# colmap/privacy_preserving_sfm

Hardware: AMD Instinct MI355X
Metric: BA iterations/sec + RANSAC hypotheses/sec, 500 cams / 200k line obs (higher is better)
Workload: dtype f64; 1 GPU; configs[2]: 500 cams / 200k line obs full BA (K1+K2+K3, MFMA Schur solve) on 1xMI355X; cams=500, points=25000, obs=200000, camera_model=SIMPLE_RADIAL, reduced_system=3000, successful_steps=2561, lm_chunk=10, submodels=1, exchange=none (independent sub-models), linear_solver=cholesky (one launch: chain workgroup + task list), cholesky_fallbacks=0

## Files before the change

### privacy_preserving_sfm_amd/csrc/chol_plan.hpp

```cpp
#pragma once
#include <algorithm>
#include <cmath>
#include <cstdint>
#include <cstdio>
#include <cstring>
#include <initializer_list>
#include <utility>
#include <vector>

#include "switches.hpp"

#ifdef __HIPCC__
#define PP_PLAN_HD __host__ __device__ __forceinline__
#else
#define PP_PLAN_HD inline
#endif

namespace ppsfm {

constexpr int kMaxChains = 16;
struct ChainRanges { int32_t n; int32_t begin[kMaxChains]; int32_t end[kMaxChains]; int32_t post[kMaxChains]; };
inline ChainRanges OneChain(int T) { ChainRanges cr; std::memset(&cr, 0, sizeof(cr)); cr.n = 1; cr.end[0] = T; return cr; }

PP_PLAN_HD void TriIndex(int t, int* row, int* col) {
  int r = (int)((sqrt(8.0 * t + 1.0) - 1.0) * 0.5);
  while ((r + 1) * (r + 2) / 2 <= t) ++r;
  while (r * (r + 1) / 2 > t) --r;
  *row = r; *col = t - r * (r + 1) / 2;
}

constexpr int BacksubNumPairs(int T) { return T >= 7 ? (T - 3) / 2 : 0; }

constexpr int kMaxSteps = 128;
constexpr int kMaxSuper = kMaxSteps / 2 + 1;
constexpr int kScratchCounters = 2048;
enum { cSol0 = 8, cVer0 = cSol0 + kMaxChains * kMaxSteps, cSub0 = cVer0 + kMaxSuper * kMaxSuper, cScratch0 = cSub0 + kMaxSuper * kMaxSuper,
       kNumCounters = cScratch0 + kScratchCounters };
static_assert(kNumCounters * sizeof(int32_t) <= 8192 * sizeof(double), "counters exceed their part of the workspace (CholeskyWorkspaceDoubles)");
enum { kTaskPrepX = 1, kTaskPrepD = 2, kTaskSolve = 3, kTaskUpdate = 4, kTaskPairPrep = 5, kTaskMerge = 6 };
struct ChainTask { int32_t type, k, a, b, w0, w1, w2, flags, cidx, sidx, zsel, mask, slot[4]; };
constexpr int TaskSuperColumn(int32_t b) { return b & 255; }
constexpr int TaskPart(int32_t b) { return (b >> 8) & 15; }
constexpr int TaskParts(int32_t b) { return (b >> 12) & 15; }
constexpr int TaskTarget(int32_t b) { return b >> 16; }
constexpr bool TaskFirstOfChain(int32_t flags) { return (flags & 1) != 0; }
constexpr int TaskChain(int32_t flags) { return (flags >> 4) & 15; }
constexpr int32_t PackUpdate(int J, int part, int parts, int target) { return J | (part << 8) | (parts << 12) | (target << 16); }
constexpr int32_t PackFlags(bool first, int chain) { return (first ? 1 : 0) | (chain << 4); }
constexpr int kPartsTwoPanels = 8;
constexpr double kUpdateSlope = 0.3;
inline int WholeFrom(int T) { return T >= 56 ? 2 : 3; }

constexpr bool StepOwnsTile(int k, int r, int c) { return (r == k + 1 && c == k + 1) || (r == k + 2 && (c == k + 1 || c == k + 2)); }

inline int CloseTileMap(int T, uint8_t* nz) {
  for (int i = 0; i < T; ++i) nz[(size_t)i * T + i] = 1;
  std::vector<int> rows;
  for (int k = 0; k < T; ++k) {
    rows.clear();
    for (int i = k + 1; i < T; ++i) if (nz[(size_t)i * T + k]) rows.push_back(i);
    for (size_t a = 0; a < rows.size(); ++a)
      for (size_t b = 0; b <= a; ++b) nz[(size_t)rows[a] * T + rows[b]] = 1;
  }
  int count = 0;
  for (int i = 0; i < T; ++i) for (int j = 0; j <= i; ++j) count += nz[(size_t)i * T + j] ? 1 : 0;
  return count;
}

struct SparseColumnLists { std::vector<int32_t> lists; int base_rows = 0, base_sups = 0; };
inline SparseColumnLists BuildSparseColumnLists(int T, const uint8_t* nz) {
  auto has = [&](int i, int j) { return i < T && j < T && nz[(size_t)i * T + j] != 0; };
  std::vector<int32_t> rows, sups, row_off(T + 1, 0), sup_off(T + 1, 0);
  for (int k = 0; k + 1 < T; ++k) {
    row_off[k] = (int32_t)rows.size(); sup_off[k] = (int32_t)sups.size();
    for (int i = k + 3; i < T; ++i) if (has(i, k)) rows.push_back(i);
    if (k >= 1) {
      const int kp = k - 1, k1 = kp + 2, nb = T - k1, ns = (nb + 1) / 2, nsup = ns * (ns + 1) / 2 - 1;
      for (int u = 0; u < nsup; ++u) {
        int I, J;
        TriIndex(u + 1, &I, &J);
        bool any = false;
        for (int q = 0; q < 4; ++q) {
          const int bi = k1 + 2 * I + (q >> 1), bj = k1 + 2 * J + (q & 1);
          any = any || (bi < T && bj < T && bi >= bj && has(bi, kp) && has(bj, kp));
// ... 46 lines not shown
  }
  if (nz) {
    p.map.assign(nz, nz + (size_t)T * T);
    for (int c = 0; c < p.cr.n; ++c)
      for (int k = p.cr.begin[c]; k < p.cr.end[c]; ++k)
        for (int i = k; i < p.cr.end[c] && i <= k + 2; ++i) p.map[(size_t)i * T + k] = 1;
    (void)CloseTileMap(T, p.map.data());
  }
  p.time.assign(T, 0);
  for (int k = 0; k < T; ++k) {
    int t = 0;
    const int ck = p.chain_of[k];
    for (int j = 0; j < k; ++j) {
      if (!nz) { t = std::max(t, p.time[j] + 1); continue; }
      if (p.chain_of[j] == ck) { if (p.map[(size_t)k * T + j]) t = std::max(t, p.time[j] + 1); continue; }
      for (int r = k; r <= k + 2 && r < p.cr.end[ck]; ++r) if (p.map[(size_t)r * T + j]) t = std::max(t, p.time[p.cr.end[p.chain_of[j]] - 1] + 2);
    }
    p.time[k] = t;
  }
  std::vector<int> order(T);
  for (int k = 0; k < T; ++k) order[k] = k;
  std::stable_sort(order.begin(), order.end(), [&](int a, int b) { return p.time[a] < p.time[b]; });
  p.rho1.assign(T, 0);
  for (int r = 0; r < T; ++r) p.rho1[order[r]] = r + 1;
  for (int c = 0; c < p.cr.n; ++c) p.cr.post[c] = p.cr.end[c] < T ? p.rho1[p.cr.end[c] - 2] : 0;
  return p;
}

struct TaskListInfo { bool fits = true; int scratch_tiles = 0; };
class TaskListBuilder {
 public:
  TaskListBuilder(int T, const ChainPlan& plan, const PlanSwitches& ps)
      : T(T), plan(plan), nz(plan.Map()), nch(plan.cr.n), whole_from(ps.whole_from ? *ps.whole_from : WholeFrom(T)), two_panels(!nz && ps.two_panels),
        slope(ps.slope ? *ps.slope : kUpdateSlope), time(plan.time), rho1(plan.rho1), own(kMaxSuper * kMaxSuper), scratch(nch),
        solpost((size_t)nch * (T + 4), 0), rowkey((size_t)nch * (T + 4), kNone), tilekey((size_t)(T + 4) * (T + 4), kNone), stepkey(T + 4, kNone) {
    for (int I = 0; I < kMaxSuper; ++I) for (int J = 0; J < kMaxSuper; ++J) { own[I * kMaxSuper + J].cidx = cVer0 + I * kMaxSuper + J; own[I * kMaxSuper + J].sidx = cSub0 + I * kMaxSuper + J; }
  }

  std::vector<ChainTask> Build(TaskListInfo* info) {
    struct Event { int t, kind, k; };
    std::vector<Event> events;
    for (int k = 0; k + 1 < T; ++k) events.push_back({time[k], 0, k});
    for (int c = 0; c + 1 < nch; ++c) events.push_back({time[plan.cr.end[c] - 1] + 1, 1, plan.cr.end[c]});
    std::stable_sort(events.begin(), events.end(), [](const Event& a, const Event& b) { return a.t != b.t ? a.t < b.t : (a.kind != b.kind ? a.kind < b.kind : a.k < b.k); });
    for (const Event& ev : events) {
      if (ev.kind == 1) { ListUpdates(ev.k, ev.t, true); ListMerges(plan.chain_of[ev.k - 1], ev.t); continue; }
      ListChainStep(ev.k);
      if (ev.k != plan.cr.begin[plan.chain_of[ev.k]]) ListUpdates(ev.k, time[ev.k], false);
    }
    if (!nz)
      for (int gp = 0; gp < BacksubNumPairs(T); ++gp)
        for (int part = 0; part < (gp + 1 < BacksubNumPairs(T) ? 3 : 1); ++part) items.push_back({2 * gp + 2.2, {kTaskPairPrep, 2 * gp + 2, gp, part, 0, 0, 0, 0, 0, 0, -1, 0, {0, 0, 0, 0}}});
    std::stable_sort(items.begin(), items.end(), [](const Item& a, const Item& b) { return a.key < b.key; });
    std::vector<ChainTask> list(items.size());
    for (size_t i = 0; i < items.size(); ++i) list[i] = items[i].t;
    if (info) { info->fits = ok; info->scratch_tiles = slots_used; }
    return list;
  }

 private:
  static constexpr double kNone = -1e30;
  struct Item { double key; ChainTask t; };
  struct Seq { int cidx = 0, sidx = 0, listed = 0, post = 0, touched = 0; double key = -1e30; int slot[4] = {-1, -1, -1, -1}; };

  const int T;
  const ChainPlan& plan;
  const uint8_t* const nz;
  const int nch, whole_from;
  const bool two_panels;
  const double slope;
  const std::vector<int>& time;
  const std::vector<int>& rho1;
  std::vector<Seq> own;
  std::vector<std::vector<std::pair<int, Seq>>> scratch;
  int scratch_used = 0, slots_used = 0;
  bool ok = true;
  std::vector<int> solpost;
  std::vector<double> rowkey;
  std::vector<double> tilekey;
  std::vector<double> stepkey;
  std::vector<Item> items;

  bool Has(int i, int j) const { return i < T && j < T && (!nz || nz[(size_t)i * T + j] != 0); }
  double& TileKey(int r, int c) { return tilekey[(size_t)r * (T + 4) + c]; }
  int& SolPost(int c, int row) { return solpost[(size_t)c * (T + 4) + row]; }
  double& RowKey(int c, int row) { return rowkey[(size_t)c * (T + 4) + row]; }
  int VerPost(int I, int J) const { return own[I * kMaxSuper + J].post; }
  double VerKey(int I, int J) const { return own[I * kMaxSuper + J].key; }
  static double Raised(double desired, std::initializer_list<double> deps) { double k = desired; for (double d : deps) k = std::max(k, d); return k; }
  int Owner(int J) const { return plan.chain_of[std::min(2 * J, T - 1)]; }
  Seq& SeqOf(int c, int I, int J) {
    if (c == Owner(J)) return own[I * kMaxSuper + J];
    for (auto& e : scratch[c]) if (e.first == I * kMaxSuper + J) return e.second;
    Seq q;
    if (scratch_used + 2 > kScratchCounters) ok = false; else { q.cidx = cScratch0 + scratch_used; q.sidx = cScratch0 + scratch_used + 1; scratch_used += 2; }
    scratch[c].push_back({I * kMaxSuper + J, q});
    return scratch[c].back().second;
  }
  double OperandKey(double dep, int k, int I, int J, int col, bool if_nz) {
    for (int row : {2 * I, 2 * I + 1, 2 * J, 2 * J + 1})
      if (row < T && row >= k + 1 && (!if_nz || Has(row, col))) dep = std::max(dep, TileKey(row, col));
    return dep;
// ... 21 lines not shown
      SolPost(c, k + 1) = rho1[k];
    }
    for (int i = k + 3; i < T; ++i)
      if (Has(i, k)) {
        const double key = Raised(tk - 0.3, {VerKey(i >> 1, k >> 1), RowKey(c, i), step_prev});
        items.push_back({key, {kTaskSolve, k, i, 0, VerPost(i >> 1, k >> 1), rho1[k], SolPost(c, i), fl, 0, 0, -1, 0, {0, 0, 0, 0}}});
        SolPost(c, i) = rho1[k]; TileKey(i, k) = key; RowKey(c, i) = key;
      }
  }

  int CoupledTiles(int k, int I, int J) const {
    int tiles = 0;
    for (int q = 0; q < 4; ++q) {
      const int bi = 2 * I + (q >> 1), bj = 2 * J + (q & 1);
      if (bi < T && bj < T && bi >= bj && bj >= k + 1 && !StepOwnsTile(k, bi, bj) && Has(bi, k - 1) && Has(bj, k - 1)) tiles |= 1 << q;
    }
    return tiles;
  }

  void ListUpdates(int k, int ts, bool pseudo) {
    const int pc = plan.chain_of[k - 1], fl = PackFlags(false, pc);
    for (int J = (k + 1) / 2; 2 * J < T; ++J)
      for (int I = J; 2 * I < T; ++I) {
        const int tiles = CoupledTiles(k, I, J);
        if (!tiles) continue;
        Seq& sq = SeqOf(pc, I, J);
        const bool into_scratch = pc != Owner(J);
        const int zsel = into_scratch ? pc : -1;
        double dep = OperandKey(sq.key, k, I, J, k - 1, true);
        const int tJ = std::min(time[2 * J], 2 * J + 1 < T ? time[2 * J + 1] : time[2 * J]);
        const int Jt = std::max(tJ / 2, (ts + 1) / 2);
        const bool front = !pseudo && I == (k + 3) / 2 && (J == I - 1 || J == I);
        const bool far = Jt - (ts + 1) / 2 >= whole_from;
        const bool far_next = two_panels && k + 2 < T && J - (k + 2) / 2 >= whole_from;
        if (far && (k & 1) == 0 && two_panels) continue;
        if (far && far_next && (k & 1) == 1) {
          sq.listed += 1;
          dep = OperandKey(dep, k, I, J, k, false);
          const double key = Raised((k + 1) + slope * (J - 0.5 * (k + 2)), {dep});
          items.push_back({key, {kTaskUpdate, k, I, PackUpdate(J, 0, kPartsTwoPanels, sq.listed), sq.post, k + 1, k, 0, sq.cidx, sq.sidx, -1, 0, {0, 0, 0, 0}}});
          sq.post = k + 1; sq.key = key;
          continue;
        }
        const int parts = front ? 4 : (far ? 1 : 2);
        sq.listed += parts;
        const double dist = std::max(0.5 * tJ - 0.5 * (ts + 1), -0.5);
        const double key = Raised(front ? ts - 0.2 : ts + slope * dist, {dep});
        const int post = std::max(rho1[k - 1], sq.post + 1);
        const int fresh = into_scratch ? (tiles & ~sq.touched) : 0;
        if (into_scratch) for (int q = 0; q < 4; ++q) if (((fresh >> q) & 1) && sq.slot[q] < 0) sq.slot[q] = slots_used++;
        for (int q = 0; q < parts; ++q)
          items.push_back({key, {kTaskUpdate, k, I, PackUpdate(J, q, parts, sq.listed), sq.post, post, rho1[k - 1], fl, sq.cidx, sq.sidx, zsel, fresh,
                                 {sq.slot[0], sq.slot[1], sq.slot[2], sq.slot[3]}}});
        sq.post = post; sq.key = key; sq.touched |= tiles;
      }
  }

  void ListMerges(int c, int ts) {
    for (auto& e : scratch[c]) {
      const int I = e.first / kMaxSuper, J = e.first % kMaxSuper;
      Seq& z = e.second;
      Seq& o = own[e.first];
      const double key = Raised(ts + 0.05, {z.key, o.key});
      const int post = o.post + 1;
      items.push_back({key, {kTaskMerge, plan.cr.end[c], I, PackUpdate(J, 0, 0, 0), o.post, post, z.post, 0, o.cidx, z.cidx, c, z.touched, {z.slot[0], z.slot[1], z.slot[2], z.slot[3]}}});
      o.post = post; o.key = key;
    }
  }
};
inline std::vector<ChainTask> BuildTaskList(int T, const ChainPlan& plan, const PlanSwitches& ps, TaskListInfo* info = nullptr) {
  return TaskListBuilder(T, plan, ps).Build(info);
}

class TaskListReplay {
// ... 90 lines not shown
    const int I = t.a, J = TaskSuperColumn(t.b), c = t.zsel;
    if (c < 0 || c >= nch || t.cidx != cVer0 + I * kMaxSuper + J) return false;
    if (ctr[t.cidx] < t.w0 || ctr[t.sidx] < t.w2) return false;
    for (int q = 0; q < 4; ++q) {
      const int r = 2 * I + (q >> 1), cc = 2 * J + (q & 1);
      if (r >= T || cc >= T) { if ((t.mask >> q) & 1) return false; continue; }
      Bits& z = zapplied[c][(size_t)r * T + cc];
      if (((t.mask >> q) & 1) != (z.none() ? 0 : 1)) return false;
      if (!z.none() && t.slot[q] != zslot[c][(size_t)r * T + cc]) return false;
      Bits& a = Applied(r, cc);
      if ((a.w[0] & z.w[0]) || (a.w[1] & z.w[1])) return false;
      a.w[0] |= z.w[0]; a.w[1] |= z.w[1];
      z = Bits();
    }
    if (ctr[t.cidx] >= t.w1) return false;
    ctr[t.cidx] = t.w1;
    return true;
  }

  bool ScratchSlotIsOwn(const ChainTask& t, int q, int r, int c) {
    int& zs = zslot[t.zsel][(size_t)r * T + c];
    if (t.slot[q] < 0) return false;
    if (zs < 0) {
      if ((int)slot_taken.size() <= t.slot[q]) slot_taken.resize(t.slot[q] + 1, 0);
      if (slot_taken[t.slot[q]]) return false;
      slot_taken[t.slot[q]] = 1; zs = t.slot[q];
    } else if (zs != t.slot[q]) return false;
    return true;
  }

  bool Update(const ChainTask& t) {
    const int k = t.k, fc = TaskChain(t.flags);
    const int I = t.a, J = TaskSuperColumn(t.b), part = TaskPart(t.b), parts = TaskParts(t.b), target = TaskTarget(t.b);
    const bool two = parts == kPartsTwoPanels;
    if (fc != plan.chain_of[k - 1] || t.zsel >= nch || (t.zsel >= 0 && t.zsel != fc)) return false;
    if (t.zsel < 0 && (t.cidx != cVer0 + I * kMaxSuper + J || t.sidx != cSub0 + I * kMaxSuper + J)) return false;
    if (ctr[t.cidx] < t.w0) return false;
    auto row_ok = [&](int row, bool distinct) {
      if (!(distinct && row < T && row >= k + 1 && Has(row, k - 1))) return true;
      int have = Sol(fc, row);
      if (ChainStores(row, k - 1)) have = std::max(have, plan.cr.post[fc]);
      return have >= (two ? t.w2 + 1 : t.w2);
    };
    const int bi = 2 * I + (parts == 2 ? part : part >> 1), bj0 = 2 * J + (parts == 2 ? 0 : part & 1), nb = parts == 2 ? 2 : 1;
    bool rows_ok;
    if (parts == 1 || two) rows_ok = row_ok(2 * I, true) && row_ok(2 * I + 1, true) && row_ok(2 * J, J != I) && row_ok(2 * J + 1, J != I);
    else rows_ok = row_ok(bi, true) && row_ok(bj0, bj0 != bi) && row_ok(bj0 + 1, nb == 2 && bj0 + 1 != bi);
    if (!rows_ok) return false;
    for (int q = 0; q < 4; ++q) {
      const int r = 2 * I + (q >> 1), c = 2 * J + (q & 1);
      const bool mine = (parts == 1 || two) || (parts == 2 ? (q >> 1) == part : q == part);
      for (int kk = k; kk <= (two ? k + 1 : k); ++kk) {
        const bool valid = r < T && c < T && r >= c && c >= kk + 1 && !StepOwnsTile(kk, r, c) && Has(r, kk - 1) && Has(c, kk - 1);
        if (!mine || !valid) continue;
        for (int row : {r, c}) if (!Solved(row, kk - 1) && !ChainStores(row, kk - 1) && !(two && kk == k + 1)) return false;
        if ((t.zsel < 0) != (plan.chain_of[kk - 1] == plan.chain_of[c])) return false;
        Bits& a = t.zsel < 0 ? Applied(r, c) : zapplied[t.zsel][(size_t)r * T + c];
        if (t.zsel >= 0 && (((t.mask >> q) & 1) != (a.none() ? 1 : 0))) return false;
        if (t.zsel >= 0 && !ScratchSlotIsOwn(t, q, r, c)) return false;
        if (a.w[(kk - 1) >> 6] >> ((kk - 1) & 63) & 1) return false;
        SetBit(&a, kk - 1);
      }
    }
    if (++ctr[t.sidx] == target) {
      if (ctr[t.cidx] >= t.w1) return false;
      ctr[t.cidx] = t.w1;
    }
    return true;
  }

  bool Complete() {
    for (int c = 0; c + 1 < T; ++c)
      for (int r = c + 1; r < T; ++r) {
        if (!Has(r, c)) continue;
        const int e = plan.cr.end[plan.chain_of[c]];
        if (r == c + 1 && r < e) { if (!Solved(r, c) && !(c + 2 >= e && CanRun(c))) return false; }
        else if (!Solved(r, c)) return false;
      }
    for (int c = 1; c < T; ++c)
      for (int r = c; r < T; ++r) {
        for (int ch = 0; ch < nch; ++ch) if (!zapplied[ch][(size_t)r * T + c].none()) return false;
        if (!Has(r, c)) continue;
        Bits want = Coupling(r, c, c);
        auto clear = [&](int p) { if (p >= 0) want.w[p >> 6] &= ~(1ull << (p & 63)); };
        clear(c - 1); if (r <= c + 1) clear(c - 2); if (r == c) clear(c - 3);
        if (!(Applied(r, c) == want)) return false;
      }
    return true;
// ... 31 lines not shown
```

### privacy_preserving_sfm_amd/csrc/cholesky.hip

```cpp
#include <algorithm>
#include <chrono>
#include <cmath>
#include <cstdio>
#include <cstdlib>
#include <cstring>
#include <mutex>
#include <string>
#include <type_traits>
#include <utility>
#include <vector>

#include "ba_impl.hpp"
#include "chol_block.hpp"
#include "chol_plan.hpp"
#include "resource_pool.hpp"

namespace ppsfm {

__global__ __launch_bounds__(kPanelThreads) void k_potrf64(double* __restrict__ S, int ld, double* __restrict__ Minv, double* __restrict__ xs, int32_t* __restrict__ flag,
                                                           double* __restrict__ x_out, double* Lout, int32_t* __restrict__ ctr, int nctr, double* mail,
                                                           long long mail_doubles, ChainRanges cr) {
  __shared__ __attribute__((aligned(16))) double smem[2 * kNB * kLS];
  __shared__ double inv_diag[kNB];
  double* A = smem;
// ... 695 lines not shown
  TileStoreD(PP_TILE(Bc, s, ct), x, lr, g);
  if (kIsX) {
#pragma unroll
    for (int r = 0; r < 4; ++r) StoreThrough(L + row_k2 + col_k + (size_t)(16 * s + g + 4 * r) * ld + 16 * ct + lr, x[r]);
    if (!FetchMailTile<true>(Ba, mb.xsol + (size_t)k * kNB * kNB, tid, flag, s_failed)) return;
    TaskStoresDone();
    if (tid == 0) __hip_atomic_store(ctr + solbase + (k + 2), done_k, __ATOMIC_RELAXED, __HIP_MEMORY_SCOPE_AGENT);
    out = UpdateTileRegs(out, Bc, Ba, ti, tj, lr, g);
    double* mail = mb.xs + (size_t)(k + 1) * kNB * kNB;
#pragma unroll
    for (int i = 0; i < 4; ++i) StoreMail(mail + (16 * ti + g + 4 * i) * kNB + 16 * tj + lr, out[i]);
    PP_TASK_MAX(5, k);
    StoreTile(L + row_k1 + col_k, Ba, ld, tid);
    TaskStoresDone();
    if (tid == 0) __hip_atomic_store(ctr + solbase + (k + 1), done_k, __ATOMIC_RELAXED, __HIP_MEMORY_SCOPE_AGENT);
  } else {
    __syncthreads();
    double* mail = mb.ds + (size_t)(k + 1) * kNB * kNB;
    if (has_out) {
      out = UpdateTileRegs(out, Bc, Bc, di, dj, lr, g);
#pragma unroll
      for (int i = 0; i < 4; ++i) StoreMail(mail + (16 * di + g + 4 * i) * kNB + 16 * dj + lr, out[i]);
    } else {
      int ui = 0, uj = 1, rem = w - 10;
      while (rem >= 3 - ui) { rem -= 3 - ui; ++ui; }
      uj = ui + 1 + rem;
#pragma unroll
      for (int i = 0; i < 4; ++i) StoreThrough(mail + (16 * ui + g + 4 * i) * kNB + 16 * uj + lr, 0.0);
    }
    PP_TASK_MAX(6, k);
  }
}

template <bool kTwo>
__device__ __forceinline__ void UpdateSuperTile(double* S, const double* L, int ld, int kp, int T, int I, int J, double* As, double* Bs, const uint8_t* __restrict__ nz, int fresh_mask = 0, double* zpool = nullptr, const int32_t* slot = nullptr) {
  const int tid = threadIdx.x, lane = tid & 63, w = tid >> 6;
  const int lr = lane & 15, lk = lane >> 4;
  const int wi = w >> 2, wj = w & 3;
  const int k = kp + 1, bi0 = 2 * I, bj0 = 2 * J;
  const int bi = bi0 + (wi >> 1), bj = bj0 + (wj >> 1);
  const bool front = (bi == k + 1 && bj == k + 1) || (bi == k + 2 && (bj == k + 1 || bj == k + 2));
  bool valid = bi < T && bj < T && bi >= bj && bj >= k + 1 && !front;
  if (valid && nz) valid = nz[(size_t)bi * T + kp] && nz[(size_t)bj * T + kp];
  const size_t cbase = (size_t)bi * kNB * ld + (size_t)bj * kNB + (size_t)(32 * (wi & 1) + lk) * ld + 32 * (wj & 1) + lr;
  const v4f64 z = (v4f64){0.0, 0.0, 0.0, 0.0};
  v4f64 c[2][2], p[2][2] = {{z, z}, {z, z}};
  const size_t col = (size_t)kp * kNB;
  const int ra1 = bi0 + 1 < T ? bi0 + 1 : bi0, rb1 = bj0 + 1 < T ? bj0 + 1 : bj0;
  const double* s0 = L + (size_t)bi0 * kNB * ld + col; const double* s1 = L + (size_t)ra1 * kNB * ld + col;
  const double* s2 = L + (size_t)bj0 * kNB * ld + col; const double* s3 = L + (size_t)rb1 * kNB * ld + col;
  LoadTiles4(As, s0, As + kNB * kLS, s1, Bs, s2, Bs + kNB * kLS, s3, ld, tid);
  const int tq = 2 * (wi >> 1) + (wj >> 1);
  const bool fresh = (fresh_mask >> tq) & 1;
  double* Cw = S + cbase;
  size_t ldc = (size_t)ld;
  if (zpool && valid) { Cw = zpool + (size_t)slot[tq] * kNB * kNB + (size_t)(32 * (wi & 1) + lk) * kNB + 32 * (wj & 1) + lr; ldc = kNB; }
  if (valid) {
#pragma unroll
    for (int a = 0; a < 2; ++a)
#pragma unroll
      for (int b = 0; b < 2; ++b)
#pragma unroll
        for (int i = 0; i < 4; ++i) c[a][b][i] = fresh ? 0.0 : LoadCoherent(Cw + (size_t)(16 * a + 4 * i) * ldc + 16 * b);
  }
  double2 nx[kTwo ? 8 : 1];
  if (kTwo) {
#pragma unroll
    for (int it = 0; it < 2; ++it) {
      nx[it] = TileLoad2(s0 + kNB, ld, tid, it); nx[2 + it] = TileLoad2(s1 + kNB, ld, tid, it);
      nx[4 + it] = TileLoad2(s2 + kNB, ld, tid, it); nx[6 + it] = TileLoad2(s3 + kNB, ld, tid, it);
    }
  }
  __syncthreads();
  const double* ar = As + (32 * wi + lr) * kLS + lk;
  const double* br = Bs + (32 * wj + lr) * kLS + lk;
  auto products = [&]() {
#pragma unroll
    for (int kk = 0; kk < 16; ++kk) {
      const double a0v = ar[4 * kk], a1v = ar[16 * kLS + 4 * kk], b0v = br[4 * kk], b1v = br[16 * kLS + 4 * kk];
      p[0][0] = __builtin_amdgcn_mfma_f64_16x16x4f64(a0v, b0v, p[0][0], 0, 0, 0);
      p[0][1] = __builtin_amdgcn_mfma_f64_16x16x4f64(a0v, b1v, p[0][1], 0, 0, 0);
      p[1][0] = __builtin_amdgcn_mfma_f64_16x16x4f64(a1v, b0v, p[1][0], 0, 0, 0);
      p[1][1] = __builtin_amdgcn_mfma_f64_16x16x4f64(a1v, b1v, p[1][1], 0, 0, 0);
    }
  };
  if (valid) products();
  if (kTwo) {
    if (valid) {
#pragma unroll
      for (int a = 0; a < 2; ++a)
#pragma unroll
        for (int b = 0; b < 2; ++b) { c[a][b] = c[a][b] - p[a][b]; p[a][b] = z; }
    }
    __syncthreads();
#pragma unroll
    for (int it = 0; it < 2; ++it) {
      TileStore2(As, tid, it, nx[it]); TileStore2(As + kNB * kLS, tid, it, nx[2 + it]);
      TileStore2(Bs, tid, it, nx[4 + it]); TileStore2(Bs + kNB * kLS, tid, it, nx[6 + it]);
    }
    __syncthreads();
    if (valid) products();
  }
  if (valid) {
#pragma unroll
    for (int a = 0; a < 2; ++a)
#pragma unroll
      for (int b = 0; b < 2; ++b)
#pragma unroll
        for (int i = 0; i < 4; ++i)
          __hip_atomic_store(Cw + (size_t)(16 * a + 4 * i) * ldc + 16 * b, c[a][b][i] - p[a][b][i], __ATOMIC_RELAXED, __HIP_MEMORY_SCOPE_AGENT);
  }
}

__device__ __forceinline__ void UpdateTilesTask(double* S, const double* L, int ld, int kp, int bi, int bj0, bool valid0, bool valid1, double* At, double* Bt, bool fresh0 = false, bool fresh1 = false, double* z0 = nullptr, double* z1 = nullptr) {
  const int tid = threadIdx.x, lane = tid & 63, w = tid >> 6, lr = lane & 15, lk = lane >> 4;
  const int ti = w >> 2, tj = w & 3;
  const size_t col = (size_t)kp * kNB;
  const size_t cbase = (size_t)bi * kNB * ld + (size_t)bj0 * kNB + (size_t)(16 * ti + lk) * ld + 16 * tj + lr;
  const v4f64 z = (v4f64){0.0, 0.0, 0.0, 0.0};
  {
    const double2 a0 = TileLoad2(L + (size_t)bi * kNB * ld + col, ld, tid, 0), a1 = TileLoad2(L + (size_t)bi * kNB * ld + col, ld, tid, 1);
    double2 b0 = make_double2(0.0, 0.0), b1 = b0, e0 = b0, e1 = b0;
    if (valid0) { b0 = TileLoad2(L + (size_t)bj0 * kNB * ld + col, ld, tid, 0); b1 = TileLoad2(L + (size_t)bj0 * kNB * ld + col, ld, tid, 1); }
    if (valid1) { e0 = TileLoad2(L + (size_t)(bj0 + 1) * kNB * ld + col, ld, tid, 0); e1 = TileLoad2(L + (size_t)(bj0 + 1) * kNB * ld + col, ld, tid, 1); }
    TileStore2(At, tid, 0, a0); TileStore2(At, tid, 1, a1);
    if (valid0) { TileStore2(Bt, tid, 0, b0); TileStore2(Bt, tid, 1, b1); }
    if (valid1) { TileStore2(Bt + kNB * kLS, tid, 0, e0); TileStore2(Bt + kNB * kLS, tid, 1, e1); }
  }
  const size_t zoff = (size_t)(16 * ti + lk) * kNB + 16 * tj + lr;
  double* C0 = z0 ? z0 + zoff : S + cbase; double* C1 = z1 ? z1 + zoff : S + cbase + kNB;
  const size_t ld0 = z0 ? (size_t)kNB : (size_t)ld, ld1 = z1 ? (size_t)kNB : (size_t)ld;
  v4f64 c0 = z, c1 = z, p0 = z, p1 = z;
  if (valid0) {
#pragma unroll
// ... 130 lines not shown
    wl.p3 = VerCounter(ctr, i >> 1, k >> 1); wl.n3 = t.w0;
    if (!TaskWait(wl, flag, &s_failed)) return;
    PP_TASK_MIN(7, k);
    if (!SolveTask(S, L, ld, k, i, mb, flag, &s_failed, B0, B1, B2, B3, prev_nz, first)) return;
    TaskStoresDone();
    if (threadIdx.x == 0) __hip_atomic_store(ctr + solbase + i, t.w1, __ATOMIC_RELAXED, __HIP_MEMORY_SCOPE_AGENT);
    PP_TASK_MAX(9, k);
    return;
  }
  if (t.type == kTaskMerge) {
    const int I = t.a, J = t.b & 255;
    WaitList wl;
    wl.p0 = ctr + t.cidx; wl.n0 = t.w0;
    wl.p1 = ctr + t.sidx; wl.n1 = t.w2;
    if (!TaskWait(wl, flag, &s_failed)) return;
#pragma unroll
    for (int q = 0; q < 4; ++q) {
      if (!((t.mask >> q) & 1)) continue;
      const size_t base = (size_t)(2 * I + (q >> 1)) * kNB * ld + (size_t)(2 * J + (q & 1)) * kNB;
      const double* Zt = Z + (size_t)t.slot[q] * kNB * kNB;
#pragma unroll
      for (int it = 0; it < 4; ++it) {
        const int idx = (int)threadIdx.x + kPanelThreads * it, r = idx >> 6, c = idx & 63;
        const size_t o = base + (size_t)r * ld + c;
        __hip_atomic_store(S + o, LoadCoherent(S + o) + LoadCoherent(Zt + r * kNB + c), __ATOMIC_RELAXED, __HIP_MEMORY_SCOPE_AGENT);
      }
    }
    TaskStoresDone();
    if (threadIdx.x == 0) __hip_atomic_store(ctr + t.cidx, t.w1, __ATOMIC_RELAXED, __HIP_MEMORY_SCOPE_AGENT);
    return;
  }
  {
    const int I = t.a, J = TaskSuperColumn(t.b), part = TaskPart(t.b), parts = TaskParts(t.b), target = TaskTarget(t.b);
    const bool two = parts == kPartsTwoPanels;
    WaitList wl;
    wl.p0 = ctr + t.cidx; wl.n0 = t.w0;
    auto row_slot = [&](int row, bool distinct, const int32_t** p, int* n) {
      const bool used = distinct && row < T && row >= k + 1 && tile_nz(row, k - 1);
      *p = ctr + solbase + (used ? row : 0); *n = used ? (two ? t.w2 + 1 : t.w2) : 0;
    };
    const int bi = 2 * I + (parts == 2 ? part : part >> 1), bj0 = 2 * J + (parts == 2 ? 0 : part & 1), nb = parts == 2 ? 2 : 1;
    if (parts == 1 || two) {
      row_slot(2 * I, true, &wl.p1, &wl.n1); row_slot(2 * I + 1, true, &wl.p2, &wl.n2);
      row_slot(2 * J, J != I, &wl.p3, &wl.n3); row_slot(2 * J + 1, J != I, &wl.p4, &wl.n4);
    } else {
      row_slot(bi, true, &wl.p1, &wl.n1);
      row_slot(bj0, bj0 != bi, &wl.p3, &wl.n3); row_slot(bj0 + 1, nb == 2 && bj0 + 1 != bi, &wl.p4, &wl.n4);
    }
#ifdef PP_CHOL_TRACE
    const bool front = (I == (k + 3) >> 1) && (J == (k + 1) >> 1 || J == (k + 3) >> 1);
    const int fs = J == (k + 1) >> 1 ? 16 : 21;
    if (front) PP_TASK_MAX(fs, k);
    unsigned long long* wait_trace = (front && fs == 16 && part == 0 && k < 128) ? &g_wait_missing[k] : nullptr;
    if (!TaskWait(wl, flag, &s_failed, wait_trace)) return;
    if (false)
#endif
    if (!TaskWait(wl, flag, &s_failed)) return;
    PP_TASK_MIN(10, k);
#ifdef PP_CHOL_TRACE
    if (front) PP_TASK_MAX(fs + 1, k);
#endif
    auto valid = [&](int r, int c) {
      const bool own = (r == k + 1 && c == k + 1) || (r == k + 2 && (c == k + 1 || c == k + 2));
      return r < T && c < T && r >= c && c >= k + 1 && !own && tile_nz(r, k - 1) && tile_nz(c, k - 1);
    };
    const bool v0 = valid(bi, bj0), v1 = nb == 2 && valid(bi, bj0 + 1);
    const int q0 = 2 * (bi - 2 * I) + (bj0 - 2 * J);
    const int ts0 = t.slot[0], ts1 = t.slot[1], ts2 = t.slot[2], ts3 = t.slot[3];
    auto slot_of = [=](int q) { return q == 0 ? ts0 : (q == 1 ? ts1 : (q == 2 ? ts2 : ts3)); };
    const bool zs = t.zsel >= 0;
    if (parts == 1) UpdateSuperTile<false>(S, L, ld, k - 1, T, I, J, B0, B2, nz, t.mask, zs ? Z : nullptr, tasks[b - cr.n].slot);
    else if (two) UpdateSuperTile<true>(S, L, ld, k - 1, T, I, J, B0, B2, nullptr);
    else if (v0 || v1) UpdateTilesTask(S, L, ld, k - 1, bi, bj0, v0, v1, B0, B2, (t.mask >> q0) & 1, (t.mask >> (q0 + 1)) & 1,
                                       zs && v0 ? Z + (size_t)slot_of(q0) * kNB * kNB : nullptr, zs && v1 ? Z + (size_t)slot_of(q0 + 1) * kNB * kNB : nullptr);
    TaskStoresDone();
    if (threadIdx.x == 0 && __hip_atomic_fetch_add(ctr + t.sidx, 1, __ATOMIC_RELAXED, __HIP_MEMORY_SCOPE_AGENT) + 1 == target)
      __hip_atomic_store(ctr + t.cidx, t.w1, __ATOMIC_RELAXED, __HIP_MEMORY_SCOPE_AGENT);
    PP_TASK_MAX(8, k);
#ifdef PP_CHOL_TRACE
    if (front) PP_TASK_MAX(fs + 2, k);
#endif
  }
}

constexpr unsigned long long kNotReady = 0xFFFFFFFFFFFFFFFFull;
__global__ __launch_bounds__(256) void k_backsub_all(const double* __restrict__ S, int ld, int T, int rhs_row, const double* __restrict__ Linv,
                                                     double* x_out, int32_t* __restrict__ flag, const uint8_t* __restrict__ nz) {
  __shared__ double part[4][kNB];
  __shared__ double ys[kNB];
  const int tid = threadIdx.x, c = tid & 63, q = tid >> 6;
  const int j = T - 1 - (int)blockIdx.x;
  double linv[16];
  {
    const double* Lb = Linv + (size_t)j * kNB * kNB;
#pragma unroll
    for (int rr = 0; rr < 16; ++rr) linv[rr] = Lb[(16 * q + rr) * kNB + c];
  }
  double acc = 0.0;
  bool dead = false;
  for (int k = T - 1; k > j; --k) {
    if (nz && !nz[(size_t)k * T + j]) continue;
    double lt[16];
    const double* Lt = S + ((size_t)k * kNB + 16 * q) * ld + (size_t)j * kNB + c;
#pragma unroll
    for (int rr = 0; rr < 16; ++rr) lt[rr] = Lt[(size_t)rr * ld];
// ... 664 lines not shown
```

### privacy_preserving_sfm_amd/csrc/switches.hip

```cpp
#include <cstdlib>

#include "switches.hpp"

namespace ppsfm {

namespace {
int Int(const char* name, int unset) {
  const char* e = std::getenv(name);
  return e ? std::atoi(e) : unset;
}
long Long(const char* name, long unset) {
  const char* e = std::getenv(name);
  return e ? std::atol(e) : unset;
}
bool Set(const char* name) { return std::getenv(name) != nullptr; }
bool Starts(const char* name, char a, char b) {
  const char* e = std::getenv(name);
  return e && (e[0] == a || e[0] == b);
}
}

Switches ReadSwitches() {
  Switches s;
  s.chol_columns = Starts("PPSFM_CHOL_MODE", 'c', '0');
  s.chol_graph = Int("PPSFM_CHOL_GRAPH", 1) != 0;
  s.chol_small = Int("PPSFM_CHOL_SMALL", 1) != 0;
  s.chol_sparse = Int("PPSFM_CHOL_SPARSE", 1) != 0;
  s.chol_test_drop_tasks = Int("PPSFM_CHOL_TEST_DROP_TASKS", 0) != 0;
  s.backsub_pairs = Int("PPSFM_BACKSUB_PAIRS", 1) != 0;
  if (Set("PPSFM_CHOL_CHAINS")) s.plan.chains = Int("PPSFM_CHOL_CHAINS", 0);
  if (Set("PPSFM_CHOL_WHOLE_FROM")) s.plan.whole_from = Int("PPSFM_CHOL_WHOLE_FROM", 0);
  s.plan.two_panels = Int("PPSFM_CHOL_TWO_PANELS", 1) != 0;
  if (const char* e = std::getenv("PPSFM_CHOL_SLOPE")) s.plan.slope = std::atof(e);
  s.chol_debug = Set("PPSFM_CHOL_DEBUG");
  s.chol_debug_slow = Set("PPSFM_CHOL_DEBUG_SLOW");
  s.chol_plan_print = Set("PPSFM_CHOL_PLAN_PRINT");
  s.ba_linear_solver = Starts("PPSFM_BA_LINEAR_SOLVER", 'i', 'I') ? LinearSolverSwitch::Iterative
                     : (Starts("PPSFM_BA_LINEAR_SOLVER", 'd', 'D') ? LinearSolverSwitch::Direct : LinearSolverSwitch::Descriptor);
  s.ba_sparse = Int("PPSFM_BA_SPARSE", 1) != 0;
  s.ba_ordering = Starts("PPSFM_BA_ORDERING", 'n', 'N') ? OrderingSwitch::Natural
                : Starts("PPSFM_BA_ORDERING", 'r', 'R') ? OrderingSwitch::Rcm
                : Starts("PPSFM_BA_ORDERING", 'b', 'B') ? OrderingSwitch::Band : OrderingSwitch::ByChainSteps;
  if (Set("PPSFM_BA_GRAPH_ND")) s.ba_graph_nd = Int("PPSFM_BA_GRAPH_ND", 0) != 0 ? 1 : 0;
  s.ba_intr_layout = Starts("PPSFM_BA_INTR_LAYOUT", 't', 'T') ? IntrLayout::Tail : IntrLayout::Beside;
  s.ba_intr_wide = Int("PPSFM_BA_INTR_WIDE", 1) != 0;
  s.ba_pair_lists = Starts("PPSFM_BA_PAIR_LISTS", 'h', 'H') ? PairListsSwitch::Host
                  : (Starts("PPSFM_BA_PAIR_LISTS", 'd', 'D') ? PairListsSwitch::Device : PairListsSwitch::BySize);
  s.ba_chunked_pairs = Int("PPSFM_BA_CHUNKED_PAIRS", 1) != 0;
  s.ba_chunk_xcd = Int("PPSFM_BA_CHUNK_XCD", 1) != 0;
  s.ba_fused_step = Int("PPSFM_BA_FUSED_STEP", 1) != 0;
  s.ba_fused_trial_cost = Int("PPSFM_BA_FUSED_TRIAL_COST", 1) != 0;
  s.pcg_fused = Int("PPSFM_PCG_FUSED", 1) != 0;
  s.ticket_spin_us = Long("PPSFM_TICKET_SPIN_US", 1500);
  s.pcg_log = Set("PPSFM_PCG_LOG");
  s.order_debug = Set("PPSFM_ORDER_DEBUG");
  s.create_debug = Set("PPSFM_CREATE_DEBUG");
  s.pool_max_mb = Long("PPSFM_POOL_MAX_MB", 1024);
  s.pool_poison = Int("PPSFM_POOL_POISON", 0) != 0;
  return s;
}

}
```

### privacy_preserving_sfm_amd/csrc/switches.hpp

```cpp
#pragma once
#include <optional>

namespace ppsfm {

enum class LinearSolverSwitch { Descriptor, Direct, Iterative };
enum class OrderingSwitch { ByChainSteps, Natural, Rcm, Band };
enum class PairListsSwitch { BySize, Host, Device };
enum class IntrLayout { Beside, Tail };

struct PlanSwitches {
  std::optional<int> chains, whole_from;
  bool two_panels = true;
  std::optional<double> slope;
  bool operator==(const PlanSwitches& o) const { return chains == o.chains && whole_from == o.whole_from && two_panels == o.two_panels && slope == o.slope; }
};

struct Switches {
  bool chol_columns = false;
  bool chol_graph = true, chol_small = true, chol_sparse = true, chol_test_drop_tasks = false, backsub_pairs = true;
  PlanSwitches plan;
  bool chol_debug = false, chol_debug_slow = false, chol_plan_print = false;
  LinearSolverSwitch ba_linear_solver = LinearSolverSwitch::Descriptor;
  bool ba_sparse = true;
  OrderingSwitch ba_ordering = OrderingSwitch::ByChainSteps;
  int ba_graph_nd = -1;
  IntrLayout ba_intr_layout = IntrLayout::Beside;
  bool ba_intr_wide = true;
  PairListsSwitch ba_pair_lists = PairListsSwitch::BySize;
  bool ba_chunked_pairs = true, ba_chunk_xcd = true, ba_fused_step = true, ba_fused_trial_cost = true, pcg_fused = true;
  long ticket_spin_us = 1500;
  bool pcg_log = false, order_debug = false, create_debug = false;
  long pool_max_mb = 1024;
  bool pool_poison = false;
};

Switches ReadSwitches();

}
```

Baseline: 1217 LM iterations/s.

## Generalize two-panel Cholesky updates to grouping up to four panels per task

Replaces the fixed two-panel supertile update with a variable panel count (up to four), grouping consecutive far-off-diagonal update steps into one task whose kernel loops over panels and prefetches the next panel while computing the current one. The task list builder now forms groups starting at any step rather than pairing only odd steps. New switches control the maximum panel count and the depth threshold, but the default maximum stays at two. The change in pairing alignment and dependency keys alters the schedule, so it can help or hurt load balance.

```diff
diff --git a/privacy_preserving_sfm_amd/csrc/chol_plan.hpp b/privacy_preserving_sfm_amd/csrc/chol_plan.hpp
--- a/privacy_preserving_sfm_amd/csrc/chol_plan.hpp
+++ b/privacy_preserving_sfm_amd/csrc/chol_plan.hpp
@@ -48,8 +48,13 @@
 constexpr int32_t PackUpdate(int J, int part, int parts, int target) { return J | (part << 8) | (parts << 12) | (target << 16); }
 constexpr int32_t PackFlags(bool first, int chain) { return (first ? 1 : 0) | (chain << 4); }
 constexpr int kPartsTwoPanels = 8;
+constexpr int kMaxPanels = 4;
+constexpr int PartsOfPanels(int panels) { return kPartsTwoPanels + panels - 2; }
+constexpr int TaskPanels(int parts) { return parts >= kPartsTwoPanels && parts <= PartsOfPanels(kMaxPanels) ? parts - kPartsTwoPanels + 2 : 1; }
 constexpr double kUpdateSlope = 0.3;
 inline int WholeFrom(int T) { return T >= 56 ? 2 : 3; }
+inline int MaxPanels(int T) { (void)T; return 2; }
+inline int DeepFrom(int T) { (void)T; return 3; }
 
 constexpr bool StepOwnsTile(int k, int r, int c) { return (r == k + 1 && c == k + 1) || (r == k + 2 && (c == k + 1 || c == k + 2)); }
 
@@ -162,6 +167,7 @@
  public:
   TaskListBuilder(int T, const ChainPlan& plan, const PlanSwitches& ps)
       : T(T), plan(plan), nz(plan.Map()), nch(plan.cr.n), whole_from(ps.whole_from ? *ps.whole_from : WholeFrom(T)), two_panels(!nz && ps.two_panels),
+        max_panels(!two_panels ? 1 : std::max(1, std::min(kMaxPanels, ps.max_panels ? *ps.max_panels : MaxPanels(T)))), deep_from(ps.deep_from ? *ps.deep_from : DeepFrom(T)),
         slope(ps.slope ? *ps.slope : kUpdateSlope), time(plan.time), rho1(plan.rho1), own(kMaxSuper * kMaxSuper), scratch(nch),
         solpost((size_t)nch * (T + 4), 0), rowkey((size_t)nch * (T + 4), kNone), tilekey((size_t)(T + 4) * (T + 4), kNone), stepkey(T + 4, kNone) {
     for (int I = 0; I < kMaxSuper; ++I) for (int J = 0; J < kMaxSuper; ++J) { own[I * kMaxSuper + J].cidx = cVer0 + I * kMaxSuper + J; own[I * kMaxSuper + J].sidx = cSub0 + I * kMaxSuper + J; }
@@ -191,13 +197,14 @@
  private:
   static constexpr double kNone = -1e30;
   struct Item { double key; ChainTask t; };
-  struct Seq { int cidx = 0, sidx = 0, listed = 0, post = 0, touched = 0; double key = -1e30; int slot[4] = {-1, -1, -1, -1}; };
+  struct Seq { int cidx = 0, sidx = 0, listed = 0, post = 0, touched = 0; double key = -1e30; int slot[4] = {-1, -1, -1, -1}; int gfirst = 0, glast = -1; };
 
   const int T;
   const ChainPlan& plan;
   const uint8_t* const nz;
   const int nch, whole_from;
   const bool two_panels;
+  const int max_panels, deep_from;
   const double slope;
   const std::vector<int>& time;
   const std::vector<int>& rho1;
@@ -285,14 +292,23 @@
         const int Jt = std::max(tJ / 2, (ts + 1) / 2);
         const bool front = !pseudo && I == (k + 3) / 2 && (J == I - 1 || J == I);
         const bool far = Jt - (ts + 1) / 2 >= whole_from;
-        const bool far_next = two_panels && k + 2 < T && J - (k + 2) / 2 >= whole_from;
-        if (far && (k & 1) == 0 && two_panels) continue;
-        if (far && far_next && (k & 1) == 1) {
+        if (max_panels > 1) {
+          if (k <= sq.glast && k != sq.glast - 1) continue;
+          if (k > sq.glast) {
+            int P = 1;
+            if (far) while (P < max_panels && k + P + 1 < T && J - (k + P + 1) / 2 >= whole_from) ++P;
+            if (P > 2 && J - (k + 1) / 2 < deep_from) P = 2;
+            if (P > 1) { sq.gfirst = k; sq.glast = k + P - 1; }
+            if (P > 2) continue;
+          }
+        }
+        if (k == sq.glast - 1) {
+          const int kf = sq.gfirst, kl = sq.glast;
           sq.listed += 1;
-          dep = OperandKey(dep, k, I, J, k, false);
-          const double key = Raised((k + 1) + slope * (J - 0.5 * (k + 2)), {dep});
-          items.push_back({key, {kTaskUpdate, k, I, PackUpdate(J, 0, kPartsTwoPanels, sq.listed), sq.post, k + 1, k, 0, sq.cidx, sq.sidx, -1, 0, {0, 0, 0, 0}}});
-          sq.post = k + 1; sq.key = key;
+          for (int col = kf - 1; col < kl; ++col) dep = OperandKey(dep, kf, I, J, col, false);
+          const double key = Raised(kl + slope * (J - 0.5 * (kl + 1)), {dep});
+          items.push_back({key, {kTaskUpdate, kf, I, PackUpdate(J, 0, PartsOfPanels(kl - kf + 1), sq.listed), sq.post, kl, kf, 0, sq.cidx, sq.sidx, -1, 0, {0, 0, 0, 0}}});
+          sq.post = kl; sq.key = key;
           continue;
         }
         const int parts = front ? 4 : (far ? 1 : 2);
@@ -449,7 +465,9 @@
   bool Update(const ChainTask& t) {
     const int k = t.k, fc = TaskChain(t.flags);
     const int I = t.a, J = TaskSuperColumn(t.b), part = TaskPart(t.b), parts = TaskParts(t.b), target = TaskTarget(t.b);
-    const bool two = parts == kPartsTwoPanels;
+    const int panels = TaskPanels(parts);
+    const bool two = panels > 1;
+    if (two && (nz || t.zsel >= 0 || k + panels - 1 >= T)) return false;
     if (fc != plan.chain_of[k - 1] || t.zsel >= nch || (t.zsel >= 0 && t.zsel != fc)) return false;
     if (t.zsel < 0 && (t.cidx != cVer0 + I * kMaxSuper + J || t.sidx != cSub0 + I * kMaxSuper + J)) return false;
     if (ctr[t.cidx] < t.w0) return false;
@@ -457,7 +475,7 @@
       if (!(distinct && row < T && row >= k + 1 && Has(row, k - 1))) return true;
       int have = Sol(fc, row);
       if (ChainStores(row, k - 1)) have = std::max(have, plan.cr.post[fc]);
-      return have >= (two ? t.w2 + 1 : t.w2);
+      return have >= t.w2 + panels - 1;
     };
     const int bi = 2 * I + (parts == 2 ? part : part >> 1), bj0 = 2 * J + (parts == 2 ? 0 : part & 1), nb = parts == 2 ? 2 : 1;
     bool rows_ok;
@@ -467,10 +485,10 @@
     for (int q = 0; q < 4; ++q) {
       const int r = 2 * I + (q >> 1), c = 2 * J + (q & 1);
       const bool mine = (parts == 1 || two) || (parts == 2 ? (q >> 1) == part : q == part);
-      for (int kk = k; kk <= (two ? k + 1 : k); ++kk) {
+      for (int kk = k; kk < k + panels; ++kk) {
         const bool valid = r < T && c < T && r >= c && c >= kk + 1 && !StepOwnsTile(kk, r, c) && Has(r, kk - 1) && Has(c, kk - 1);
         if (!mine || !valid) continue;
-        for (int row : {r, c}) if (!Solved(row, kk - 1) && !ChainStores(row, kk - 1) && !(two && kk == k + 1)) return false;
+        for (int row : {r, c}) if (!Solved(row, kk - 1) && !ChainStores(row, kk - 1) && !(two && kk > k)) return false;
         if ((t.zsel < 0) != (plan.chain_of[kk - 1] == plan.chain_of[c])) return false;
         Bits& a = t.zsel < 0 ? Applied(r, c) : zapplied[t.zsel][(size_t)r * T + c];
         if (t.zsel >= 0 && (((t.mask >> q) & 1) != (a.none() ? 1 : 0))) return false;
diff --git a/privacy_preserving_sfm_amd/csrc/cholesky.hip b/privacy_preserving_sfm_amd/csrc/cholesky.hip
--- a/privacy_preserving_sfm_amd/csrc/cholesky.hip
+++ b/privacy_preserving_sfm_amd/csrc/cholesky.hip
@@ -751,8 +751,8 @@
   }
 }
 
-template <bool kTwo>
-__device__ __forceinline__ void UpdateSuperTile(double* S, const double* L, int ld, int kp, int T, int I, int J, double* As, double* Bs, const uint8_t* __restrict__ nz, int fresh_mask = 0, double* zpool = nullptr, const int32_t* slot = nullptr) {
+template <bool kDeep>
+__device__ __forceinline__ void UpdateSuperTile(double* S, const double* L, int ld, int kp, int T, int I, int J, double* As, double* Bs, const uint8_t* __restrict__ nz, int fresh_mask = 0, double* zpool = nullptr, const int32_t* slot = nullptr, int np = 1) {
   const int tid = threadIdx.x, lane = tid & 63, w = tid >> 6;
   const int lr = lane & 15, lk = lane >> 4;
   const int wi = w >> 2, wj = w & 3;
@@ -782,14 +782,16 @@
 #pragma unroll
         for (int i = 0; i < 4; ++i) c[a][b][i] = fresh ? 0.0 : LoadCoherent(Cw + (size_t)(16 * a + 4 * i) * ldc + 16 * b);
   }
-  double2 nx[kTwo ? 8 : 1];
-  if (kTwo) {
-#pragma unroll
-    for (int it = 0; it < 2; ++it) {
-      nx[it] = TileLoad2(s0 + kNB, ld, tid, it); nx[2 + it] = TileLoad2(s1 + kNB, ld, tid, it);
-      nx[4 + it] = TileLoad2(s2 + kNB, ld, tid, it); nx[6 + it] = TileLoad2(s3 + kNB, ld, tid, it);
-    }
-  }
+  double2 nx[kDeep ? 8 : 1];
+  auto request = [&](int pn) {
+    uint32_t t = (uint32_t)tid;
+    asm volatile("" : "+v"(t));
+    const uint32_t boff = ((t >> 5) * (uint32_t)ld + 2u * (t & 31)) * (uint32_t)sizeof(double);
+    auto at = [&](const double* base, int it) { return *reinterpret_cast<const double2*>(reinterpret_cast<const char*>(base + (size_t)pn * kNB + (size_t)(32 * it) * ld) + boff); };
+#pragma unroll
+    for (int it = 0; it < 2; ++it) { nx[it] = at(s0, it); nx[2 + it] = at(s1, it); nx[4 + it] = at(s2, it); nx[6 + it] = at(s3, it); }
+  };
+  if (kDeep) request(1);
   __syncthreads();
   const double* ar = As + (32 * wi + lr) * kLS + lk;
   const double* br = Bs + (32 * wj + lr) * kLS + lk;
@@ -804,21 +806,26 @@
     }
   };
   if (valid) products();
-  if (kTwo) {
-    if (valid) {
-#pragma unroll
-      for (int a = 0; a < 2; ++a)
-#pragma unroll
-        for (int b = 0; b < 2; ++b) { c[a][b] = c[a][b] - p[a][b]; p[a][b] = z; }
-    }
-    __syncthreads();
-#pragma unroll
-    for (int it = 0; it < 2; ++it) {
-      TileStore2(As, tid, it, nx[it]); TileStore2(As + kNB * kLS, tid, it, nx[2 + it]);
-      TileStore2(Bs, tid, it, nx[4 + it]); TileStore2(Bs + kNB * kLS, tid, it, nx[6 + it]);
-    }
-    __syncthreads();
-    if (valid) products();
+  if (kDeep) {
+#pragma unroll
+    for (int pn = 1; pn < kMaxPanels; ++pn) {
+      if (pn >= np) break;
+      if (valid) {
+#pragma unroll
+        for (int a = 0; a < 2; ++a)
+#pragma unroll
+          for (int b = 0; b < 2; ++b) { c[a][b] = c[a][b] - p[a][b]; p[a][b] = z; }
+      }
+      __syncthreads();
+#pragma unroll
+      for (int it = 0; it < 2; ++it) {
+        TileStore2(As, tid, it, nx[it]); TileStore2(As + kNB * kLS, tid, it, nx[2 + it]);
+        TileStore2(Bs, tid, it, nx[4 + it]); TileStore2(Bs + kNB * kLS, tid, it, nx[6 + it]);
+      }
+      if (pn + 1 < np) request(pn + 1);
+      __syncthreads();
+      if (valid) products();
+    }
   }
   if (valid) {
 #pragma unroll
@@ -1015,12 +1022,13 @@
   }
   {
     const int I = t.a, J = TaskSuperColumn(t.b), part = TaskPart(t.b), parts = TaskParts(t.b), target = TaskTarget(t.b);
-    const bool two = parts == kPartsTwoPanels;
+    const int panels = TaskPanels(parts);
+    const bool two = panels > 1;
     WaitList wl;
     wl.p0 = ctr + t.cidx; wl.n0 = t.w0;
     auto row_slot = [&](int row, bool distinct, const int32_t** p, int* n) {
       const bool used = distinct && row < T && row >= k + 1 && tile_nz(row, k - 1);
-      *p = ctr + solbase + (used ? row : 0); *n = used ? (two ? t.w2 + 1 : t.w2) : 0;
+      *p = ctr + solbase + (used ? row : 0); *n = used ? t.w2 + panels - 1 : 0;
     };
     const int bi = 2 * I + (parts == 2 ? part : part >> 1), bj0 = 2 * J + (parts == 2 ? 0 : part & 1), nb = parts == 2 ? 2 : 1;
     if (parts == 1 || two) {
@@ -1053,7 +1061,7 @@
     auto slot_of = [=](int q) { return q == 0 ? ts0 : (q == 1 ? ts1 : (q == 2 ? ts2 : ts3)); };
     const bool zs = t.zsel >= 0;
     if (parts == 1) UpdateSuperTile<false>(S, L, ld, k - 1, T, I, J, B0, B2, nz, t.mask, zs ? Z : nullptr, tasks[b - cr.n].slot);
-    else if (two) UpdateSuperTile<true>(S, L, ld, k - 1, T, I, J, B0, B2, nullptr);
+    else if (two) UpdateSuperTile<true>(S, L, ld, k - 1, T, I, J, B0, B2, nullptr, 0, nullptr, nullptr, panels);
     else if (v0 || v1) UpdateTilesTask(S, L, ld, k - 1, bi, bj0, v0, v1, B0, B2, (t.mask >> q0) & 1, (t.mask >> (q0 + 1)) & 1,
                                        zs && v0 ? Z + (size_t)slot_of(q0) * kNB * kNB : nullptr, zs && v1 ? Z + (size_t)slot_of(q0 + 1) * kNB * kNB : nullptr);
     TaskStoresDone();
diff --git a/privacy_preserving_sfm_amd/csrc/switches.hip b/privacy_preserving_sfm_amd/csrc/switches.hip
--- a/privacy_preserving_sfm_amd/csrc/switches.hip
+++ b/privacy_preserving_sfm_amd/csrc/switches.hip
@@ -31,6 +31,8 @@
   if (Set("PPSFM_CHOL_CHAINS")) s.plan.chains = Int("PPSFM_CHOL_CHAINS", 0);
   if (Set("PPSFM_CHOL_WHOLE_FROM")) s.plan.whole_from = Int("PPSFM_CHOL_WHOLE_FROM", 0);
   s.plan.two_panels = Int("PPSFM_CHOL_TWO_PANELS", 1) != 0;
+  if (Set("PPSFM_CHOL_MAX_PANELS")) s.plan.max_panels = Int("PPSFM_CHOL_MAX_PANELS", 0);
+  if (Set("PPSFM_CHOL_DEEP_FROM")) s.plan.deep_from = Int("PPSFM_CHOL_DEEP_FROM", 0);
   if (const char* e = std::getenv("PPSFM_CHOL_SLOPE")) s.plan.slope = std::atof(e);
   s.chol_debug = Set("PPSFM_CHOL_DEBUG");
   s.chol_debug_slow = Set("PPSFM_CHOL_DEBUG_SLOW");
diff --git a/privacy_preserving_sfm_amd/csrc/switches.hpp b/privacy_preserving_sfm_amd/csrc/switches.hpp
--- a/privacy_preserving_sfm_amd/csrc/switches.hpp
+++ b/privacy_preserving_sfm_amd/csrc/switches.hpp
@@ -9,10 +9,10 @@
 enum class IntrLayout { Beside, Tail };
 
 struct PlanSwitches {
-  std::optional<int> chains, whole_from;
+  std::optional<int> chains, whole_from, max_panels, deep_from;
   bool two_panels = true;
   std::optional<double> slope;
-  bool operator==(const PlanSwitches& o) const { return chains == o.chains && whole_from == o.whole_from && two_panels == o.two_panels && slope == o.slope; }
+  bool operator==(const PlanSwitches& o) const { return chains == o.chains && whole_from == o.whole_from && two_panels == o.two_panels && max_panels == o.max_panels && deep_from == o.deep_from && slope == o.slope; }
 };
 
 struct Switches {
```

After: 1217 LM iterations/s, median of 2. About the same (-0.0%).
